# songhayeong/aes-fhe

Measured on AMD Instinct MI355X. Metric: AES-128 blocks/sec (homomorphic full round) at N=2^16, L=30; 1/2/4/8 MI355X, higher is better.
Workload: dtype u64

## Files before the change

### aes-fhe_amd/csrc/engine.hip

```cpp
#include <hip/hip_runtime.h>

#include <algorithm>
#include <atomic>
#include <cstdarg>
#include <cstdlib>
#include <cstdio>
#include <cstring>
#include <map>
#include <unordered_map>
#include <memory>
#include <mutex>
#include <string>
#include <vector>

#include "../../include/aesfhe.h"
#include "kernels_ops.h"
#include "ntt256f.h"
#include "ks_fused.h"
#include "bconv_mfma.h"
#include "bconv_cols.h"
#include "basis_tables.h"
#include "bsgs_plan.h"
#include "operands.h"
#include "arena.h"
// ... 824 lines not shown
extern "C" void aesfhe_key_free(aesfhe_key* k) {
    if (!k) return;
    aesfhe_engine* e = k->eng;
    e->pool.put(k->d, k->bytes);
    delete k;
    engine_unref(e);
}
extern "C" int aesfhe_key_info(const aesfhe_key* k, int32_t* kind, uint64_t* g) {
    *kind = k->kind;
    *g = k->galois;
    return 0;
}
extern "C" uint64_t aesfhe_galois_elt(int32_t logN, int64_t rot, int32_t conj) {
    u64 M = 2ULL << logN, n = 1ULL << (logN - 1);
    if (conj) return M - 1;
    int64_t r = rot % (int64_t)n;
    if (r < 0) r += (int64_t)n;
    u64 ex = (n - (u64)r) % n;
    return h_powmod(5, ex, M);
}

static aesfhe_key* key_new(aesfhe_engine* e, int kind, size_t words) {
    auto* k = new aesfhe_key;
    k->eng = e;
    e->refs++;
    k->kind = kind;
    k->galois = 0;
    k->keyseed = 0;
    k->bytes = words * 8;
    k->d = (u64*)pool_get(e, k->bytes);
    return k;
}

static void sample_small_ntt(aesfhe_engine* e, u64* dst, int nprimes, u64 key, int kind) {
    Span s = span_s(dst, 0, nprimes, std::min(nprimes, e->Lp1), 0, e->Lp1);
    s.pstride = (long)nprimes * e->N;
    hipLaunchKernelGGL(k_sample_small, dim3((e->N / 8 + 255) / 256), dim3(256), 0, e->stream, s, e->ck, key, kind, e->q, e->logN, e->Lp1, nprimes);
    ntt(e, s, s, nprimes, false);
}

extern "C" int aesfhe_key_secret(aesfhe_engine* e, uint64_t seed, aesfhe_key** out) {
    API_BEGIN
    aesfhe_key* k = key_new(e, 0, (size_t)e->np * e->N);
    k->keyseed = derive(e->seed, seed);
    sample_small_ntt(e, k->d, e->np, derive(k->keyseed, 1), 0);
    *out = k;
    API_END
}

extern "C" int aesfhe_key_public(aesfhe_engine* e, const aesfhe_key* sk, aesfhe_key** out) {
    API_BEGIN
    if (!sk || sk->kind != 0) throw_err(AESFHE_EARG, "public key needs a secret key");
    const int N = e->N, nq = e->Lp1;
    aesfhe_key* k = key_new(e, 1, (size_t)2 * nq * N);
    k->keyseed = sk->keyseed;
    u64* b = k->d;
    u64* a = k->d + (size_t)nq * N;
    Span sa = span_s(a, 0, nq, nq, 0, e->Lp1);
    hipLaunchKernelGGL(k_sample_uniform, dim3((N / 8 + 255) / 256, nq), dim3(256), 0, e->stream, sa, e->ck, derive(sk->keyseed, 2), e->q, e->logN, e->Lp1);
    Tmp et(e, (size_t)nq * N);
    sample_small_ntt(e, et.p, nq, derive(sk->keyseed, 3), 1);
    hipLaunchKernelGGL(k_key_combine, dim3(N / 256, nq), dim3(256), 0, e->stream, a, sk->d, et.p, (const u64*)nullptr, (const u64*)nullptr, 0, 0, b, e->q, e->qinv, e->logN);
    HIPC(hipGetLastError());
    *out = k;
    API_END
}

static aesfhe_key* make_ksk_t(aesfhe_engine* e, const u64* starget, u64 keyseed, const u64* sprime, int kind,
                              u64 g, u64 salt) {
    const int N = e->N, np = e->np;
    aesfhe_key* k = key_new(e, kind, (size_t)e->dnum * 2 * np * N);
    k->galois = g;
    k->keyseed = keyseed;
    k->ndig = e->dnum;
    u64 base = derive(derive(keyseed, 4 + (u64)kind), g);
    if (salt) base = derive(base, salt);
    Tmp et(e, (size_t)np * N);
    for (int d = 0; d < e->dnum; d++) {
        u64* kb = k->d + ((size_t)d * 2 + 0) * np * N;
        u64* ka = k->d + ((size_t)d * 2 + 1) * np * N;
        Span sa = span_s(ka, 0, np, e->Lp1, 0, e->Lp1);
        hipLaunchKernelGGL(k_sample_uniform, dim3((N / 8 + 255) / 256, np), dim3(256), 0, e->stream, sa, e->ck, derive(base, 2 * (u64)d), e->q, e->logN, e->Lp1);
        sample_small_ntt(e, et.p, np, derive(base, 2 * (u64)d + 1), 1);
        int lo = d * e->A, hi = std::min(lo + e->A, e->Lp1);
        hipLaunchKernelGGL(k_key_combine, dim3(N / 256, np), dim3(256), 0, e->stream, (const u64*)ka, starget, et.p, sprime, e->pmod, lo, hi, kb, e->q, e->qinv, e->logN);
    }
    HIPC(hipGetLastError());
    return k;
}
static aesfhe_key* make_ksk(aesfhe_engine* e, const aesfhe_key* sk, const u64* sprime, int kind, u64 g,
                            u64 salt = 0) {
    return make_ksk_t(e, sk->d, sk->keyseed, sprime, kind, g, salt);
}

extern "C" int aesfhe_key_relin(aesfhe_engine* e, const aesfhe_key* sk, aesfhe_key** out) {
    API_BEGIN
    if (!sk || sk->kind != 0) throw_err(AESFHE_EARG, "relinearization key needs a secret key");
    Tmp s2(e, (size_t)e->np * e->N);
    hipLaunchKernelGGL(k_square, dim3(e->N / 256, e->np), dim3(256), 0, e->stream, sk->d, s2.p, e->q, e->qinv, e->logN);
    *out = make_ksk(e, sk, s2.p, 2, 0);
    API_END
}

extern "C" int aesfhe_key_galois(aesfhe_engine* e, const aesfhe_key* sk, uint64_t g, aesfhe_key** out) {
    API_BEGIN
    if (!sk || sk->kind != 0) throw_err(AESFHE_EARG, "galois key needs a secret key");
    if (!(g & 1) || g >= 2ULL * e->N) throw_err(AESFHE_EARG, "bad galois element");
    Tmp sg(e, (size_t)e->np * e->N);
    Span src = span_s(sk->d, 0, e->np, e->Lp1, 0, e->Lp1), dst = span_s(sg.p, 0, e->np, e->Lp1, 0, e->Lp1);
    hipLaunchKernelGGL(k_galois, dim3(e->N / 256, e->np), dim3(256), 0, e->stream, src, dst, (u64)g, e->logN, e->Lp1);
    *out = make_ksk(e, sk, sg.p, 3, g);
    API_END
}

extern "C" int aesfhe_key_galois_hoisted(aesfhe_engine* e, const aesfhe_key* sk, uint64_t g, aesfhe_key** out) {
    API_BEGIN
    if (!sk || sk->kind != 0) throw_err(AESFHE_EARG, "galois key needs a secret key");
    if (!(g & 1) || g >= 2ULL * e->N) throw_err(AESFHE_EARG, "bad galois element");
    const u64 M = 2ULL * e->N;
    u64 ginv = 1;
// ... 75 lines not shown
    const size_t per = c->bytes / c->B;
    HIPC(hipMemcpyAsync(dst, (const char*)c->d + per * start, per * count, hipMemcpyDeviceToDevice, e->stream));
    HIPC(hipStreamSynchronize(e->stream));
    API_END
}
extern "C" int aesfhe_ct_import_device(aesfhe_engine* e, const void* src, int32_t B, int32_t np, int32_t level,
                                       aesfhe_ct** out) {
    API_BEGIN
    if (!src || B < 1 || np < 1 || np > 3 || level < 0 || level > e->L) throw_err(AESFHE_EARG, "bad shape");
    CtPtr c = ct_new(e, B, np, level);
    HIPC(hipMemcpyAsync(c->d, src, c->bytes, hipMemcpyDeviceToDevice, e->stream));
    HIPC(hipStreamSynchronize(e->stream));
    *out = c.release();
    API_END
}

static size_t key_words(const aesfhe_engine* e, int kind) {
    switch (kind) {
        case 0: return (size_t)e->np * e->N;
        case 1: return (size_t)2 * e->Lp1 * e->N;
        case 2: case 3: case 5: return (size_t)e->dnum * 2 * e->np * e->N;
        default: return 0;
    }
}
extern "C" int aesfhe_key_export(aesfhe_engine* e, const aesfhe_key* k, int32_t* kind, uint64_t* galois,
                                 uint64_t* keyseed, int64_t* words, uint64_t* out) {
    API_BEGIN
    if (!k) throw_err(AESFHE_EARG, "null key");
    *kind = k->kind;
    *galois = k->galois;
    *keyseed = k->keyseed;
    *words = (int64_t)(k->bytes / 8);
    if (out) {
        HIPC(hipMemcpyAsync(out, k->d, k->bytes, hipMemcpyDeviceToHost, e->stream));
        HIPC(hipStreamSynchronize(e->stream));
    }
    API_END
}
extern "C" int aesfhe_key_import(aesfhe_engine* e, int32_t kind, uint64_t galois, uint64_t keyseed,
                                 const uint64_t* in, int64_t words, aesfhe_key** out) {
    API_BEGIN
    size_t want = key_words(e, kind);
    if (!in || !want) throw_err(AESFHE_EARG, "unknown key kind %d", kind);
    int ndig = 0;
    if (kind == 2 || kind == 3 || kind == 5) {
        const size_t dw = (size_t)2 * e->np * e->N;
        if (words > 0 && (size_t)words % dw == 0 && (size_t)words / dw >= 1 && (size_t)words / dw <= (size_t)e->dnum)
            want = (size_t)words, ndig = (int)((size_t)words / dw);
    }
    if ((size_t)words != want) throw_err(AESFHE_EARG, "key of kind %d needs %zu words, got %lld", kind, want, (long long)words);
    aesfhe_key* k = key_new(e, kind, want);
    k->galois = galois;
    k->keyseed = keyseed;
    k->ndig = ndig;
    HIPC(hipMemcpyAsync(k->d, in, want * 8, hipMemcpyHostToDevice, e->stream));
    HIPC(hipStreamSynchronize(e->stream));
    *out = k;
    API_END
}
extern "C" int aesfhe_key_trim(aesfhe_engine* e, aesfhe_key* k, int32_t max_level) {
    API_BEGIN
    if (!k || k->ndig < 1) throw_err(AESFHE_EARG, "only switching keys (relinearization, galois, hoisted rotation) can be trimmed");
    if (max_level < 0 || max_level > e->L) throw_err(AESFHE_EARG, "bad level %d", max_level);
    const int nd = (max_level + 1 + e->A - 1) / e->A;
    if (nd < k->ndig) {
        const size_t bytes = (size_t)nd * 2 * e->np * e->N * 8;
        u64* d = (u64*)pool_get(e, bytes);
        HIPC(hipMemcpyAsync(d, k->d, bytes, hipMemcpyDeviceToDevice, e->stream));
        e->pool.put(k->d, k->bytes);
        k->d = d;
        k->bytes = bytes;
        k->ndig = nd;
    }
    API_END
}
static CtPtr ct_copy_new(aesfhe_engine* e, const aesfhe_ct* c) {
    CtPtr r = ct_new(e, c->B, c->np, c->level);
    HIPC(hipMemcpyAsync(r->d, c->d, c->bytes, hipMemcpyDeviceToDevice, e->stream));
    r->is_zero = c->is_zero;
    return r;
}
extern "C" int aesfhe_ct_copy(aesfhe_engine* e, const aesfhe_ct* c, aesfhe_ct** out) {
    API_BEGIN
    *out = ct_copy_new(e, c).release();
    API_END
}
extern "C" int aesfhe_ct_slice(aesfhe_engine* e, const aesfhe_ct* c, int32_t start, int32_t count, aesfhe_ct** out) {
    API_BEGIN
// ... 698 lines not shown
    a.scs = acs;
    a.dst = dst;
    a.dbs = 2 * kN;
    a.dcs = kN;
    a.nc = 2;
    a.ns = e->K + r;
    a.s_nq = r;
    a.s_q0 = lk + 1;
    a.s_p0 = e->Lp1;
    a.sinvf = ysrc ? nullptr : t.invf;
    a.einv = t.einv;
    a.nt = lk + 1;
    a.skip0 = lk + 1;
    a.skipn = 0;
    a.tl_l = lk;
    a.Lp1 = e->Lp1;
    a.tab = t.tab;
    a.corr = t.corr;
    a.pc = e->bc_pc;
    a.qall = e->q;
    a.qinvall = e->qinv;
    return a;
}

template <bool VC>
static void launch_bconv_cols_t(aesfhe_engine* e, const BconvArgs& a, int nz, int nslots) {
    const int nstep = (nslots + 3) / 4, ntile = (a.nt + 3) / 4;
    if (e->logN != 16 || nstep < 1 || nstep > 4 || ntile < 1 || (16 * nz) % 8)
        throw_err(AESFHE_EUNSUPPORTED, "fused base conversion of %d slots to %d targets", nslots, a.nt);
    if (!a.src || !a.dst || !a.tab || !a.corr || !a.pc || (VC && !a.einv))
        throw_err(AESFHE_EUNSUPPORTED, "fused base conversion with a missing table");
    const dim3 g((unsigned)(16 * nz * ntile));
    const Tabs T = e->tabs();
#define BCC(S) hipLaunchKernelGGL((k_bconv_cols<S, true, VC, 1>), g, dim3(256), 0, e->stream, a, T, ntile)
    switch (nstep) {
        case 1: BCC(1); break;
        case 2: BCC(2); break;
        case 3: BCC(3); break;
        default: BCC(4); break;
    }
#undef BCC
    HIPC(hipGetLastError());
}
static void launch_bconv_cols(aesfhe_engine* e, const BconvArgs& a, int nz) { launch_bconv_cols_t<false>(e, a, nz, a.ns); }

static std::vector<unsigned short> bsgs_block_order(int logN, const std::vector<u64>& gal) {
    std::vector<unsigned short> ord;
    if (!aesfhe::bsgs_block_order(logN, std::vector<uint64_t>(gal.begin(), gal.end()), ord))
        throw_err(AESFHE_EUNSUPPORTED, "bsgs block order is not a permutation");
    return ord;
}

static int ks_beta(const aesfhe_engine* e, int l) {
    const int beta = (l + 1 + e->A - 1) / e->A;
    if (beta > 12) throw_err(AESFHE_EUNSUPPORTED, "more than 12 key-switch digits");
    return beta;
}
static void check_key_digits(aesfhe_engine* e, const aesfhe_key* k, int l) {
    if (k && k->ndig > 0 && ks_beta(e, l) > k->ndig)
        throw_err(AESFHE_ELEVEL, "key trimmed to %d digits cannot switch at level %d (%d digits)", k->ndig, l, ks_beta(e, l));
}

static void ks_modup(aesfhe_engine* e, const u64* d, long dbs, int B, int l, u64* ext, bool cols_only = false,
                     const Opnd* pa = nullptr, const Opnd* pb = nullptr, const u64* fac = nullptr) {
    const int N = e->N, K = e->K, ne = l + 1 + K;
    const long lN = (long)(l + 1) * N, neN = (long)ne * N;
    const int beta = ks_beta(e, l);
// ... 1281 lines not shown
```

### aes-fhe_amd/csrc/ext/engine_ext.hip

```cpp
#include "../engine.hip"

#include "../../../include/aesfhe_ext.h"
#include "kernels_expand.h"
#include "kernels_lincomb_int.h"
#include "kernels_ptb.h"
#include "kernels_wire.h"

struct aesfhe_ptb {
    aesfhe_engine* eng;
    int B, level;
    u64* d;
    size_t bytes;
};

static const int kMaxGridZ = 65535;

extern "C" int aesfhe_ptb_create_device(aesfhe_engine* e, const int64_t* co, int32_t B, int32_t level, aesfhe_ptb** out) {
    API_BEGIN
    if (!e || !out) throw_err(AESFHE_EARG, "null argument");
    if (!co || ((uintptr_t)co & 15)) throw_err(AESFHE_EARG, "coefficient buffer must be a 16-byte aligned device pointer");
    if (level < 0 || level > e->L) throw_err(AESFHE_EARG, "bad plaintext level");
    if (B < 1 || B > kMaxGridZ) throw_err(AESFHE_EARG, "plaintext batch %d not in 1..%d", B, kMaxGridZ);
    const int N = e->N, nl = level + 1;
    struct PtbFree {
// ... 257 lines not shown
                           (const u64*)e->q, e->logN, (unsigned long long*)flag.p);
    }
    HIPC(hipGetLastError());
    u64 bad = 0;
    HIPC(hipMemcpyAsync(&bad, flag.p, 8, hipMemcpyDeviceToHost, e->stream));
    HIPC(hipStreamSynchronize(e->stream));
    if (bad) throw_err(AESFHE_EARG, "blob holds a residue that is not below its prime");
}

extern "C" int aesfhe_key_pack(aesfhe_engine* e, const aesfhe_key* k, const aesfhe_key* target, const uint8_t* seed, void* dst,
                               int64_t* bytes) {
    API_BEGIN
    if (!e || !k || !bytes) throw_err(AESFHE_EARG, "null argument");
    if (k->eng != e) throw_err(AESFHE_EARG, "key of another engine");
    if (target) {
        if (!seed) throw_err(AESFHE_EARG, "seeded packing needs 32 seed bytes");
        if (k->kind == 0) throw_err(AESFHE_EARG, "a secret key has no mask to seed");
        if (target->eng != e || target->kind != 0) throw_err(AESFHE_EARG, "seeded packing needs the secret key the rows are encrypted under");
    }
    const WireDims d = wire_dims(e);
    WireHeader h = wire_header_of(e, d);
    h.type = kWireKey, h.kind = k->kind, h.ndig = (uint32_t)k->ndig, h.galois = k->galois, h.keyseed = k->keyseed;
    h.npoly = k->kind == 0 ? 1 : 2;
    h.level = (k->kind == 1 ? e->Lp1 : e->np) - 1;
    WireShape s;
    if (!wire_pack_begin(e, d, h, s, seed, target != nullptr, dst, bytes)) return AESFHE_OK;
    if ((size_t)s.groups * s.polys * s.nl * e->N * 8 != k->bytes) throw_err(AESFHE_EARG, "key block of %zu bytes does not match its kind", k->bytes);
    u64 gal = 1;
    if (target && k->kind == 5) {
        const u64 M = 2ULL * e->N;
        for (u64 x = 1;; x = x * k->galois % M)
            if (x * k->galois % M == 1) { gal = x; break; }
    }
    wire_pack_run(e, h, s, k->d, target ? target->d : nullptr, gal, dst);
    API_END
}

extern "C" int aesfhe_ct_pack(aesfhe_engine* e, const aesfhe_ct* c, const aesfhe_key* sk, const uint8_t* seed, void* dst, int64_t* bytes) {
    API_BEGIN
    if (!e || !c || !bytes) throw_err(AESFHE_EARG, "null argument");
    if (c->eng != e) throw_err(AESFHE_EARG, "ciphertext of another engine");
    const bool seeded = sk != nullptr && !c->is_zero;
    if (sk) {
        if (!seed) throw_err(AESFHE_EARG, "seeded packing needs 32 seed bytes");
        if (sk->eng != e || sk->kind != 0) throw_err(AESFHE_EARG, "seeded packing needs the secret key");
        if (seeded && c->np != 2) throw_err(AESFHE_EDEGREE, "Input ciphertext should have 2 polynomials");
    }
    const WireDims d = wire_dims(e);
    WireHeader h = wire_header_of(e, d);
    h.type = kWireCt, h.batch = c->B, h.npoly = c->np, h.level = c->level, h.zero = c->is_zero ? 1 : 0;
    WireShape s;
    if (!wire_pack_begin(e, d, h, s, seed, seeded, dst, bytes)) return AESFHE_OK;
    wire_pack_run(e, h, s, c->d, seeded ? sk->d : nullptr, 1, dst);
    API_END
}

static void wire_unpack_begin(const aesfhe_engine* e, const void* src, int64_t bytes, uint32_t type, WireHeader& h, WireShape& s) {
    if (e->logN < kWireMinLogN) throw_err(AESFHE_EARG, "the wire format needs N >= 1024");
    const std::string err = wire_parse((const uint8_t*)src, bytes, wire_dims(e), h, s);
    if (!err.empty()) throw_err(AESFHE_EARG, "cannot unpack: %s", err.c_str());
    if (h.type != type) throw_err(AESFHE_EARG, "the blob holds a %s", h.type == kWireKey ? "key" : "ciphertext");
}

extern "C" int aesfhe_key_unpack(aesfhe_engine* e, const void* src, int64_t bytes, aesfhe_key** out) {
    API_BEGIN
    if (!e || !src || !out) throw_err(AESFHE_EARG, "null argument");
    WireHeader h;
    WireShape s;
    wire_unpack_begin(e, src, bytes, kWireKey, h, s);
    struct KeyFree {
        void operator()(aesfhe_key* k) const { aesfhe_key_free(k); }
    };
    std::unique_ptr<aesfhe_key, KeyFree> k(key_new(e, h.kind, (size_t)s.groups * s.polys * s.nl * e->N));
    k->galois = h.galois, k->keyseed = h.keyseed, k->ndig = (int)h.ndig;
    wire_unpack_run(e, h, s, src, k->d);
    *out = k.release();
    API_END
}

extern "C" int aesfhe_ct_unpack(aesfhe_engine* e, const void* src, int64_t bytes, aesfhe_ct** out) {
    API_BEGIN
    if (!e || !src || !out) throw_err(AESFHE_EARG, "null argument");
    WireHeader h;
    WireShape s;
    wire_unpack_begin(e, src, bytes, kWireCt, h, s);
    if (h.zero) {
        *out = ct_zero_new(e, h.batch, h.npoly, h.level).release();
        return AESFHE_OK;
    }
    CtPtr c = ct_new(e, h.batch, h.npoly, h.level);
    wire_unpack_run(e, h, s, src, c->d);
    *out = c.release();
    API_END
}
```

### aes-fhe_amd/csrc/kernels.h

```cpp
#pragma once
#include <hip/hip_runtime.h>

#include <cstdint>

#define AESFHE_HD __host__ __device__
#include "ckks_host.h"

namespace aesfhe {

constexpr int kMaxPrimes = 96;
constexpr double kBigPrime = 4398046511104.0;

__device__ __forceinline__ u64 add_m(u64 a, u64 b, u64 q) {
    u64 s = a + b;
    return s >= q ? s - q : s;
}
__device__ __forceinline__ u64 sub_m(u64 a, u64 b, u64 q) { return a >= b ? a - b : a + q - b; }

__device__ __forceinline__ u64 fix_m(u64 r, u64 q) {
    int64_t s = (int64_t)r;
    s = s < 0 ? s + (int64_t)q : s;
    s = s >= (int64_t)q ? s - (int64_t)q : s;
    return (u64)s;
}

__device__ __forceinline__ double u2d(u64 a) {
    return __longlong_as_double((long long)(a | 0x4330000000000000ULL)) - 4503599627370496.0;
}
__device__ __forceinline__ u64 rint_u(double x_times, double scale) {
    return (u64)__double_as_longlong(__builtin_fma(x_times, scale, 4503599627370496.0)) & 0xFFFFFFFFFFFFFULL;
}

__device__ __forceinline__ u64 mul_m(u64 a, u64 b, u64 q, double qinv) {
    const u64 qh = rint_u(u2d(a) * u2d(b), qinv);
    return fix_m(a * b - qh * q, q);
}
__device__ __forceinline__ u64 mul_w(u64 a, u64 w, double wq, u64 q) {
    const u64 qh = rint_u(u2d(a), wq);
    int64_t r = (int64_t)(a * w - qh * q);
    r += (r >> 63) & (int64_t)q;
    return (u64)r;
}

constexpr double kMagic52 = 6755399441055744.0;
__device__ __forceinline__ double fmul_rem(double a, double w, double wq, double q) {
    const double p = a * w;
    const double pl = __builtin_fma(a, w, -p);
    const double qh = __builtin_rint(a * wq);
    const double u = __builtin_fma(-qh, q, p);
    return u + pl;
}
__device__ __forceinline__ double fmul_rem_r(double a, double w, double wq, double q) {
    return fmul_rem(a, w, wq, q);
}
__device__ __forceinline__ double fmul_remq(double a, double w, double qi, double q) {
    const double p = a * w;
    const double pl = __builtin_fma(a, w, -p);
    const double qh = __builtin_rint(p * qi);
    const double u = __builtin_fma(-qh, q, p);
    return u + pl;
}
// ... 196 lines not shown
```

### aes-fhe_amd/csrc/kernels_ops.h

```cpp
#pragma once
#include "kernels.h"

namespace aesfhe {

__device__ __forceinline__ u64 red_m(u64 x, u64 q, double qinv) {
    u64 qh = (u64)((double)x * qinv);
    return fix_m(x - qh * q, q);
}

struct Opnd {
    const u64* ptr;
    long bs;
    long ps;
    int np;
    int bmask = -1;
};

__device__ const u64 kZeroWord = 0;
__device__ __forceinline__ u64 opnd_get(const Opnd& o, int b, int p, int l, int k, int logN) {
    const bool has = o.ptr && p < o.np;
    return *(has ? o.ptr + (long)(b & o.bmask) * o.bs + (long)p * o.ps + ((long)l << logN) + k : &kZeroWord);
}

struct Out {
// ... 261 lines not shown

__global__ void k_rescale_finish_g(const u64* __restrict__ c, long cps, const u64* __restrict__ t,
                                   u64* const* __restrict__ outs, long ops, int np, int Bg, int l,
                                   const u64* __restrict__ qs, const u64* __restrict__ inv,
                                   const double* __restrict__ invf, int logN) {
    const int k = blockIdx.x * blockDim.x + threadIdx.x;
    const int i = blockIdx.y, P = blockIdx.z;
    const int g = P / (Bg * np), rem = P - g * Bg * np;
    const u64 q = qs[i];
    u64 cv = c[(long)P * cps + ((long)i << logN) + k];
    u64 tv = t[(((long)P * l + i) << logN) + k];
    outs[g][(long)rem * ops + ((long)i << logN) + k] = mul_w(sub_m(cv, tv, q), inv[i], invf[i], q);
}

template <int BM>
__global__ void k_ks_inner_all(const u64* __restrict__ d, long dbs, const u64* __restrict__ ext,
                               long exs, long exj, const u64* __restrict__ key, long kdig,
                               long kcomp, u64* __restrict__ acc, long abs_, long acs, int B,
                               int beta, int K, int l, const u64* __restrict__ qall,
                               const double* __restrict__ qinvall, int Lp1, Opnd addend,
                               const double* __restrict__ pmodf, int logN, int accum) {
    const int k = blockIdx.x * blockDim.x + threadIdx.x;
    const int t = blockIdx.y;
    const int pid = t <= l ? t : Lp1 + (t - l - 1);
    const double q = (double)qall[pid];
    const double qi = qinvall[pid];
    const int own = t <= l ? t / K : -1;
    double kb[BM], ka[BM];
#pragma unroll
    for (int j = 0; j < BM; j++) {
        kb[j] = ka[j] = 0.0;
        if (j < beta) {
            const long ko = (long)j * kdig + ((long)pid << logN) + k;
            kb[j] = u2d(key[ko]);
            ka[j] = u2d(key[ko + kcomp]);
        }
    }
#pragma unroll 4
    for (int bb = 0; bb < B; bb++) {
        double s0 = 0.0, s1 = 0.0;
#pragma unroll
        for (int j = 0; j < BM; j++) {
            if (j < beta) {
                const double e = u2d((j == own) ? d[(long)bb * dbs + ((long)t << logN) + k]
                                                : ext[(long)j * exj + (long)bb * exs + ((long)t << logN) + k]);
                s0 += fmul_remq(e, kb[j], qi, q);
                s1 += fmul_remq(e, ka[j], qi, q);
                if ((j & 3) == 3) {
                    s0 = fred(s0, q, qi);
                    s1 = fred(s1, q, qi);
                }
            }
        }
        if (pmodf && t <= l) {
            const double f = pmodf[t], w = tw_w(f, q);
            s0 = fred(s0, q, qi) + fmul_rem(u2d(opnd_get(addend, bb, 0, t, k, logN)), w, f, q);
            s1 = fred(s1, q, qi) + fmul_rem(u2d(opnd_get(addend, bb, 1, t, k, logN)), w, f, q);
        }
        u64* a0 = acc + (long)bb * abs_ + ((long)t << logN) + k;
        if (accum) {
            s0 += u2d(a0[0]);
            s1 += u2d(a0[acs]);
        }
        a0[0] = fcanon(s0, q, qi);
        a0[acs] = fcanon(s1, q, qi);
    }
}

template <int BM, int KC>
__global__ void k_ks_inner_multi(const u64* __restrict__ d, long dbs, const u64* __restrict__ ext,
                                 long exs, long exj, const u64* const* __restrict__ keys, int nk, long kdig,
                                 long kcomp, u64* const* __restrict__ accs, long abs_, long acs, int B,
                                 int beta, int K, int l, const u64* __restrict__ qall,
                                 const double* __restrict__ qinvall, int Lp1, Opnd addend,
                                 const double* __restrict__ pmodf, int logN) {
    const int k = blockIdx.x * blockDim.x + threadIdx.x;
    const int t = blockIdx.y;
    const int pid = t <= l ? t : Lp1 + (t - l - 1);
    const double q = (double)qall[pid];
    const double qi = qinvall[pid];
    const int own = t <= l ? t / K : -1;
    const bool pm = pmodf && t <= l;
    const double f = pm ? pmodf[t] : 0.0, fw = pm ? tw_w(f, q) : 0.0;
    for (int i0 = 0; i0 < nk; i0 += KC) {
        double kb[KC][BM], ka[KC][BM];
#pragma unroll
        for (int ii = 0; ii < KC; ii++) {
#pragma unroll
            for (int j = 0; j < BM; j++) {
                const bool ok = i0 + ii < nk && j < beta;
                const u64* kp = keys[ok ? i0 + ii : 0] + (long)j * kdig + ((long)pid << logN) + k;
                kb[ii][j] = u2d(*(ok ? kp : &kZeroWord));
                ka[ii][j] = u2d(*(ok ? kp + kcomp : &kZeroWord));
            }
        }
#pragma unroll 1
        for (int bb = 0; bb < B; bb++) {
            double e[BM];
#pragma unroll
            for (int j = 0; j < BM; j++)
                e[j] = u2d(*(j >= beta ? &kZeroWord
                             : (j == own) ? d + (long)bb * dbs + ((long)t << logN) + k
                                          : ext + (long)j * exj + (long)bb * exs + ((long)t << logN) + k));
            double ad0 = 0.0, ad1 = 0.0;
            if (pm) {
                ad0 = fmul_rem(u2d(opnd_get(addend, bb, 0, t, k, logN)), fw, f, q);
                ad1 = fmul_rem(u2d(opnd_get(addend, bb, 1, t, k, logN)), fw, f, q);
            }
#pragma unroll
            for (int ii = 0; ii < KC; ii++) {
                if (i0 + ii >= nk) break;
                double s0 = 0.0, s1 = 0.0;
#pragma unroll
                for (int j = 0; j < BM; j++) {
                    if (j < beta) {
                        s0 += fmul_remq(e[j], kb[ii][j], qi, q);
                        s1 += fmul_remq(e[j], ka[ii][j], qi, q);
                        if ((j & 3) == 3) {
                            s0 = fred(s0, q, qi);
                            s1 = fred(s1, q, qi);
                        }
                    }
                }
                if (pm) {
                    s0 = fred(s0, q, qi) + ad0;
                    s1 = fred(s1, q, qi) + ad1;
// ... 142 lines not shown
            ulonglong2 w;
            w.x = v[e] >= 0 ? (u64)v[e] : q - (u64)(-v[e]);
            w.y = v[e + 1] >= 0 ? (u64)v[e + 1] : q - (u64)(-v[e + 1]);
            *(ulonglong2*)&out[k0 + e] = w;
        }
    }
}

__global__ void k_coeffs_res(const i64* __restrict__ co, u64* __restrict__ out, int nl,
                             const u64* __restrict__ qs, int logN) {
    const int k = blockIdx.x * blockDim.x + threadIdx.x;
    const int l = blockIdx.y, bb = blockIdx.z;
    const i64 v = co[((long)bb << logN) + k];
    const u64 q = qs[l];
    u64 r;
    if (v >= 0) r = (u64)v % q;
    else r = q - 1 - ((u64)(-(v + 1)) % q);
    out[(((long)bb * nl + l) << logN) + k] = r;
}

__global__ void k_key_combine(const u64* __restrict__ a, const u64* __restrict__ s,
                              const u64* __restrict__ e, const u64* __restrict__ sp,
                              const u64* __restrict__ pmod, int lo, int hi, u64* __restrict__ out,
                              const u64* __restrict__ qall, const double* __restrict__ qinvall,
                              int logN) {
    const int k = blockIdx.x * blockDim.x + threadIdx.x;
    const int pid = blockIdx.y;
    const long off = ((long)pid << logN) + k;
    const u64 q = qall[pid];
    const double qi = qinvall[pid];
    u64 v = add_m(sub_m(0, mul_m(a[off], s[off], q, qi), q), e[off], q);
    if (sp && pid >= lo && pid < hi) v = add_m(v, mul_m(pmod[pid], sp[off], q, qi), q);
    out[off] = v;
}

__global__ void k_enc_pk(const u64* __restrict__ vem, const u64* __restrict__ pk0,
                         const u64* __restrict__ pk1, u64* __restrict__ ct, int nl,
                         const u64* __restrict__ qs, const double* __restrict__ qinv, int logN) {
    const int k = blockIdx.x * blockDim.x + threadIdx.x;
    const int l = blockIdx.y, bb = blockIdx.z;
    const u64 q = qs[l];
    const double qi = qinv[l];
    const long lo = ((long)l << logN) + k;
    const long step = (long)nl << logN;
    const u64* base = vem + (long)bb * 4 * step + lo;
    u64 v = base[0], e0 = base[step], e1 = base[2 * step], m = base[3 * step];
    u64* c = ct + (long)bb * 2 * step + lo;
    c[0] = add_m(add_m(mul_m(v, pk0[lo], q, qi), e0, q), m, q);
    c[step] = add_m(mul_m(v, pk1[lo], q, qi), e1, q);
}

__global__ void k_enc_sk(const u64* __restrict__ vem, const u64* __restrict__ s,
                         u64* __restrict__ ct, int nl, const u64* __restrict__ qs,
                         const double* __restrict__ qinv, ChaKey K, const u64* __restrict__ keys, int logN) {
    const int k0 = (blockIdx.x * blockDim.x + threadIdx.x) * 8;
    if (k0 >= (1 << logN)) return;
    const int l = blockIdx.y, bb = blockIdx.z;
    const u64 q = qs[l];
    const double qi = qinv[l];
    const long step = (long)nl << logN;
    uint32_t o[16];
    chacha20_block(K, keys[bb], (((u64)l << logN) + k0) >> 3, o);
#pragma unroll
    for (int e = 0; e < 8; e++) {
        const long lo = ((long)l << logN) + k0 + e;
        const u64* base = vem + (long)bb * 4 * step + lo;
// ... 578 lines not shown
            for (int j = 0; j < GM; j++) {
                acc0[u][j] += fmul_remq(f0, wv[j], qi, q);
                acc1[u][j] += fmul_remq(f1, wv[j], qi, q);
            }
        }
    };
    int i = 0;
    if (!keys[0]) {
        double wv[GM], e0[BB], e1[BB];
#pragma unroll
        for (int j = 0; j < GM; j++) wv[j] = pt_word(j, 0);
#pragma unroll
        for (int u = 0; u < BB; u++) {
            e0[u] = isq ? fmul_rem(u2d(*(isq ? c0r[u] + k : &kZeroWord)), pw, pf, q) : 0.0;
            e1[u] = isq ? fmul_rem(u2d(*(isq ? c1r[u] + k : &kZeroWord)), pw, pf, q) : 0.0;
        }
        add_terms(e0, e1, wv);
        i = 1;
    }
    int nsum = 1;
#pragma unroll 1
    for (; i < nb; i += PB) {
        double kb[PB][BM], ka[PB][BM], x[PB][BB][BM], c0v[PB][BB], wv[PB][GM];
#pragma unroll
        for (int p = 0; p < PB; p++) {
            const int ii = min(i + p, nb - 1);
            const bool live = i + p < nb;
            const u64 g = gal[ii];
            const long src = __brev((unsigned)((((g * ek) & (M - 1)) - 1) >> 1)) >> (32 - logN);
            const u64* kp = keys[ii];
#pragma unroll
            for (int d = 0; d < BM; d++) {
                const u64* kk = kp + (long)min(d, beta - 1) * kdig + ((long)pid << logN) + src;
                kb[p][d] = u2d(kk[0]);
                ka[p][d] = u2d(kk[kcomp]);
            }
#pragma unroll
            for (int j = 0; j < GM; j++) wv[p][j] = live ? pt_word(j, ii) : 0.0;
#pragma unroll
            for (int u = 0; u < BB; u++) {
#pragma unroll
                for (int d = 0; d < BM; d++)
                    x[p][u][d] = u2d(*(d == own ? c1r[u] + src : er[u] + (long)min(d, beta - 1) * exj + src));
                c0v[p][u] = u2d(*(isq ? c0r[u] + src : &kZeroWord));
            }
        }
#pragma unroll
        for (int p = 0; p < PB; p++) {
            double e0[BB], e1[BB];
#pragma unroll
            for (int u = 0; u < BB; u++) {
                double a0 = isq ? fmul_rem(c0v[p][u], pw, pf, q) : 0.0, a1 = 0.0;
#pragma unroll
                for (int d = 0; d < BM; d++) {
                    if (d < beta) {
                        a0 += fmul_remq(x[p][u][d], kb[p][d], qi, q);
                        a1 += fmul_remq(x[p][u][d], ka[p][d], qi, q);
                        if ((d & 3) == 3) {
                            a0 = fred(a0, q, qi);
                            a1 = fred(a1, q, qi);
                        }
                    }
                }
                e0[u] = a0;
                e1[u] = a1;
            }
            add_terms(e0, e1, wv[p]);
        }
// ... 27 lines not shown
```

### aes-fhe_amd/csrc/ks_fused.h

```cpp
#pragma once
#include "kernels_ops.h"
#include "ntt256f.h"

#include <type_traits>

namespace aesfhe {

__device__ __forceinline__ int r8p(int e) { return e + (e >> 3); }

__device__ __forceinline__ void wave_lds_sync() {
    __builtin_amdgcn_fence(__ATOMIC_RELEASE, "wavefront");
    __builtin_amdgcn_wave_barrier();
    __builtin_amdgcn_fence(__ATOMIC_ACQUIRE, "wavefront");
}

template <bool BIG>
using KsBig = std::integral_constant<bool, BIG>;
template <class Big>
__device__ __forceinline__ void row_ntt8_stages(double (&x)[8], double* sr, int L, int rt, const double* W, double q,
                                                double qi, Big big);
__device__ __forceinline__ void row_ntt8_fwd(double (&x)[8], const u64* rp, double* sr, int L, int rt,
                                             const double* W, double q, double qi, bool big) {
#pragma unroll
    for (int r = 0; r < 8; r++) x[r] = ld_d(&rp[L + 32 * r]);
// ... 93 lines not shown
    const int eb = 32 * (L >> 2) + (L & 3);
#pragma unroll
    for (int r = 0; r < 8; r++) x[r] = sr[r8p(eb + 4 * r)];
#pragma unroll
    for (int st = 5; st >= 3; st--) {
        const int ml = 1 << st, h = 4 >> (st - 3), nj = ml >> 3;
        const int base = ml + (L >> 2) * nj;
#pragma unroll
        for (int j = 0; j < nj; j++) {
            const double w = W[base + j];
#pragma unroll
            for (int k = 0; k < h; k++) gs_f<BIG>(x[j * 2 * h + k], x[j * 2 * h + k + h], w, q, qi);
        }
    }
    wave_lds_sync();
#pragma unroll
    for (int r = 0; r < 8; r++) sr[r8p(eb + 4 * r)] = x[r];
    wave_lds_sync();
#pragma unroll
    for (int r = 0; r < 8; r++) x[r] = sr[r8p(L + 32 * r)];
#pragma unroll
    for (int st = 2; st >= 0; st--) {
        const int ml = 1 << st, h = 4 >> st;
#pragma unroll
        for (int j = 0; j < ml; j++) {
            const double w = W[ml + j];
#pragma unroll
            for (int k = 0; k < h; k++) gs_f<BIG>(x[j * 2 * h + k], x[j * 2 * h + k + h], w, q, qi);
        }
    }
    wave_lds_sync();
}

template <bool FMA, bool HAS_C, bool BIG>
__device__ __forceinline__ void ks_prod_prologue(double (&a0)[8], double (&a1)[8], const u64* kp, long kcomp,
                                                 const u64* xa, long aps, const u64* xb, long bps, const u64* xc,
                                                 long cps, double wv, double f, double fal, double fC, double fK,
                                                 double q, double qi) {
    static_assert(FMA || !HAS_C, "the addend ciphertext belongs to the multiply-add form");
    double x0[8], x1[8], y0[8], y1[8], kb[8], ka[8];
#pragma unroll
    for (int r = 0; r < 8; r++) {
        x0[r] = u2d(xa[32 * r]);
        x1[r] = u2d(xa[aps + 32 * r]);
        y0[r] = u2d(xb[32 * r]);
        y1[r] = u2d(xb[bps + 32 * r]);
        if constexpr (!FMA) {
            kb[r] = u2d(kp[32 * r]);
            ka[r] = u2d(kp[32 * r + kcomp]);
        }
    }
#pragma unroll
    for (int r = 0; r < 8; r++) {
        if constexpr (FMA) {
            kb[r] = u2d(kp[32 * r]);
            ka[r] = u2d(kp[32 * r + kcomp]);
        }
        double p0 = fmul_remq(x0[r], y0[r], qi, q);
        double p1 = fmul_remq(x0[r], y1[r], qi, q) + fmul_remq(x1[r], y0[r], qi, q);
        double p2 = fmul_remq(x1[r], y1[r], qi, q);
        if constexpr (FMA) {
            p0 = fmul_remq(p0, fal, qi, q) + fK;
            p1 = fmul_remq(p1, fal, qi, q);
            p2 = fmul_remq(p2, fal, qi, q);
            if constexpr (HAS_C) {
                p0 += fmul_remq(u2d(xc[32 * r]), fC, qi, q);
                p1 += fmul_remq(u2d(xc[cps + 32 * r]), fC, qi, q);
            }
        }
        a0[r] = fmul_rem(p0, wv, f, q) + fmul_remq(p2, kb[r], qi, q);
        a1[r] = fmul_rem(p1, wv, f, q) + fmul_remq(p2, ka[r], qi, q);
        if constexpr (BIG) {
            a0[r] = fred(a0[r], q, qi);
            a1[r] = fred(a1[r], q, qi);
        }
    }
}

struct KsFin {
    const u64* conv;
    long cbs, cps;
    u64* out;
    long obs, ops;
    const double* dinvf;
    Opnd2 add;
};
template <int G, int R = 256, bool PROD = false, int EPI = 0>
__global__ __launch_bounds__(256, 4) void k_nttf_rows_ks(const u64* __restrict__ d, long dbs,
                                                      const u64* __restrict__ ext, long exs, long exj,
                                                      const u64* __restrict__ key, long kdig, long kcomp,
                                                      u64* __restrict__ acc, long abs_, long acs, int B,
                                                      int beta, int K, int l, int ne, Tabs T, Opnd addend,
                                                      const double* __restrict__ pmodf, int accum, Opnd pb,
                                                      const u64* __restrict__ fac, Opnd pc, int t0, int nt,
                                                      KsFin fin) {
    static_assert(G == 1 && !PROD && EPI == 0, "the accumulating giants' kernel: the other forms are k_nttf_rows_ks_p's");
    __shared__ double s[8 * 288 + 8 * 256];
    const int nbg = (B + G - 1) / G;
    const int id = blockIdx.x, x8 = id & 7, rest = id >> 3;
    const int b0 = (rest % nbg) * G, pair = (rest / nbg) * 8 + x8;
    constexpr int RB = R / 8;
    constexpr int LOGN = R == 256 ? 16 : 17;
    const int tq = pair / RB, rb = pair - tq * RB;
    if (tq >= nt) return;
    const int t = t0 + tq;
    const int pid = t <= l ? t : T.Lp1 + (t - l - 1);
    const int own = t <= l ? t / K : -1;
    const int tid = threadIdx.x, L = tid & 31, rl = tid >> 5;
// ... 15 lines not shown
    const long roff = ((long)t << LOGN) + (long)row * 256 + L;
    double a0[G][8], a1[G][8];
#pragma unroll
    for (int g = 0; g < G; g++) {
        const int bb = b0 + g;
#pragma unroll
        for (int r = 0; r < 8; r++) a0[g][r] = a1[g][r] = 0.0;
        if (bb >= B) continue;
        if (pmodf && t <= l && addend.ptr) {
            const double f = pmodf[t], w = tw_w(f, q);
            const u64* xa = addend.ptr + (long)bb * addend.bs + roff;
            if (addend.np > 0) {
#pragma unroll
                for (int r = 0; r < 8; r++) a0[g][r] = fmul_rem(u2d(xa[32 * r]), w, f, q);
            }
            if (addend.np > 1) {
#pragma unroll
                for (int r = 0; r < 8; r++) a1[g][r] = fmul_rem(u2d(xa[addend.ps + 32 * r]), w, f, q);
            }
        }
        if (accum) {
            const u64* o0 = acc + (long)bb * abs_ + roff;
#pragma unroll
            for (int r = 0; r < 8; r++) {
                a0[g][r] = fred(a0[g][r] + u2d(o0[32 * r]), q, qi);
                a1[g][r] = fred(a1[g][r] + u2d(o0[acs + 32 * r]), q, qi);
            }
        }
    }
    int nsum = 0;
#pragma unroll 1
    for (int j = 0; j < beta; j++) {
        const u64* kp = key + (long)j * kdig + ((long)pid << LOGN) + (long)row * 256 + L;
        u64 kbw[8], kaw[8];
#pragma unroll
        for (int r = 0; r < 8; r++) {
            kbw[r] = kp[32 * r];
            kaw[r] = kp[32 * r + kcomp];
        }
#pragma unroll
        for (int g = 0; g < G; g++) {
            const int bb = b0 + g;
            if (bb >= B) break;
            double v[8];
            if (j == own) {
                const u64* dp = d + (long)bb * dbs + roff;
#pragma unroll
                for (int r = 0; r < 8; r++) v[r] = u2d(dp[32 * r]);
            } else {
                row_ntt8_fwd(v, ext + (long)j * exj + (long)bb * exs + ((long)t << LOGN) + (long)row * 256, sr, L, 1,
                             tw, q, qi, big);
            }
#pragma unroll
            for (int r = 0; r < 8; r++) {
                const double kb = u2d(kbw[r]), ka = u2d(kaw[r]);
                a0[g][r] += fmul_remq(v[r], kb, qi, q);
                a1[g][r] += fmul_remq(v[r], ka, qi, q);
            }
        }
        if (big && (++nsum & 3) == 0) {
#pragma unroll
            for (int g = 0; g < G; g++)
#pragma unroll
                for (int r = 0; r < 8; r++) {
                    a0[g][r] = fred(a0[g][r], q, qi);
                    a1[g][r] = fred(a1[g][r], q, qi);
                }
        }
    }
#pragma unroll
    for (int g = 0; g < G; g++) {
        const int bb = b0 + g;
        if (bb >= B) break;
        u64* o0 = acc + (long)bb * abs_ + roff;
#pragma unroll
        for (int r = 0; r < 8; r++) {
            __builtin_nontemporal_store(fcanon(a0[g][r], q, qi), &o0[32 * r]);
            __builtin_nontemporal_store(fcanon(a1[g][r], q, qi), &o0[acs + 32 * r]);
        }
    }
}

typedef __attribute__((address_space(3))) void ks_lds_void;
__device__ __forceinline__ void ks_dma_rows(const u64* g, double* lds_wave, int lane) {
#pragma unroll
    for (int k = 0; k < 4; k++)
        __builtin_amdgcn_global_load_lds((const void*)(g + 128 * k + 2 * lane), (ks_lds_void*)(lds_wave + 128 * k), 16, 0, 0);
}
__device__ __forceinline__ void ks_dma_wait() {
    asm volatile("s_waitcnt vmcnt(0)" ::: "memory");
// ... 30 lines not shown
    const double q = (double)T.q[pid], qi = T.qinv[pid];
    const double* W = T.psid + ((long)pid << LOGN);
    double* sr = s + rl * 288;
    double* tw = s + 8 * 288 + rl * 256;
    double* ebw = s + 8 * 288 + 8 * 256 + w * 512;
    const double* er = ebw + (rl & 1) * 256;
    const long woff = ((long)t << LOGN) + (long)(rb * 8 + 2 * w) * 256;
    auto next_digit = [&](int j) { return j + 1 == own ? j + 2 : j + 1; };
    int jn = next_digit(-1);
    if (jn < beta) ks_dma_rows(ext + (long)jn * exj + (long)bb * exs + woff, ebw, lane);
#pragma unroll
    for (int m = 0; m < 8; m++) {
        const int e = L + 32 * m;
        if (e > 0) {
            const int ml = 1 << (31 - __clz(e));
            tw[e] = W[(long)ml * (R + row) + (e - ml)];
        }
    }
    const long roff = ((long)t << LOGN) + (long)row * 256 + L;
    auto body = [&](auto big) {
        constexpr bool BIG = decltype(big)::value;
        double a0[8], a1[8];
#pragma unroll
        for (int r = 0; r < 8; r++) a0[r] = a1[r] = 0.0;
        if (PROD && t <= l) {
            const double f = pmodf[t], wv = tw_w(f, q);
            const u64* kp = key + (long)own * kdig + ((long)pid << LOGN) + (long)row * 256 + L;
            const u64* xa = addend.ptr + (long)(bb & addend.bmask) * addend.bs + roff;
            const u64* xb = pb.ptr + (long)(bb & pb.bmask) * pb.bs + roff;
            const u64* xc = pc.ptr ? pc.ptr + (long)(bb & pc.bmask) * pc.bs + roff : xb;
            if (fac) {
                const double fal = (double)fac[3 * t], fC = (double)fac[3 * t + 1], fK = (double)fac[3 * t + 2];
                if (pc.ptr)
                    ks_prod_prologue<true, true, BIG>(a0, a1, kp, kcomp, xa, addend.ps, xb, pb.ps, xc, pc.ps, wv, f, fal, fC,
                                                      fK, q, qi);
                else
                    ks_prod_prologue<true, false, BIG>(a0, a1, kp, kcomp, xa, addend.ps, xb, pb.ps, xc, pc.ps, wv, f, fal,
                                                       fC, fK, q, qi);
            } else {
                ks_prod_prologue<false, false, BIG>(a0, a1, kp, kcomp, xa, addend.ps, xb, pb.ps, xc, pc.ps, wv, f, 0.0, 0.0,
                                                    0.0, q, qi);
            }
        } else if (!PROD) {
            if (pmodf && t <= l && addend.ptr) {
                const double f = pmodf[t], wv = tw_w(f, q);
                const u64* xa = addend.ptr + (long)bb * addend.bs + roff;
                if (addend.np > 0) {
#pragma unroll
                    for (int r = 0; r < 8; r++) a0[r] = fmul_rem(u2d(xa[32 * r]), wv, f, q);
                }
                if (addend.np > 1) {
#pragma unroll
                    for (int r = 0; r < 8; r++) a1[r] = fmul_rem(u2d(xa[addend.ps + 32 * r]), wv, f, q);
                }
            }
            if (own >= 0 && own < beta) {
                const u64* kp = key + (long)own * kdig + ((long)pid << LOGN) + (long)row * 256 + L;
                const u64* dp = d + (long)bb * dbs + roff;
#pragma unroll
                for (int r = 0; r < 8; r++) {
                    const double v = u2d(dp[32 * r]), kb = u2d(kp[32 * r]), ka = u2d(kp[32 * r + kcomp]);
                    a0[r] += fmul_remq(v, kb, qi, q);
                    a1[r] += fmul_remq(v, ka, qi, q);
                }
            }
        }
        if (accum) {
            const u64* o0 = acc + (long)bb * abs_ + roff;
#pragma unroll
            for (int r = 0; r < 8; r++) {
                a0[r] = fred(a0[r] + u2d(o0[32 * r]), q, qi);
                a1[r] = fred(a1[r] + u2d(o0[acs + 32 * r]), q, qi);
            }
        } else if (BIG) {
#pragma unroll
            for (int r = 0; r < 8; r++) {
                a0[r] = fred(a0[r], q, qi);
                a1[r] = fred(a1[r], q, qi);
            }
        }
        wave_lds_sync();
        int nsum = 0;
        const long coff = ((long)t << LOGN) + (long)(rb * 8 + 2 * w) * 256;
#pragma unroll 1
        while (jn < beta) {
            const int j = jn;
            ks_dma_wait();
            double v[8];
#pragma unroll
            for (int r = 0; r < 8; r++) v[r] = er[L + 32 * r];
            ks_lds_reads_done();
            jn = next_digit(j);
            if constexpr (FIN)
                ks_dma_rows(jn < beta ? ext + (long)jn * exj + (long)bb * exs + woff : fin.conv + (long)bb * fin.cbs + coff,
                            ebw, lane);
            else if (jn < beta) ks_dma_rows(ext + (long)jn * exj + (long)bb * exs + woff, ebw, lane);
            const u64* kp = key + (long)j * kdig + ((long)pid << LOGN) + (long)row * 256 + L;
            u64 kbw[8], kaw[8];
#pragma unroll
            for (int r = 0; r < 8; r++) {
                kbw[r] = kp[32 * r];
                kaw[r] = kp[32 * r + kcomp];
            }
            row_ntt8_stages(v, sr, L, 1, tw, q, qi, big);
#pragma unroll
            for (int r = 0; r < 8; r++) {
                const double kb = u2d(kbw[r]), ka = u2d(kaw[r]);
                a0[r] += fmul_remq(v[r], kb, qi, q);
                a1[r] += fmul_remq(v[r], ka, qi, q);
            }
            if (BIG && (++nsum & 3) == 0) {
#pragma unroll
                for (int r = 0; r < 8; r++) {
                    a0[r] = fred(a0[r], q, qi);
                    a1[r] = fred(a1[r], q, qi);
                }
            }
        }
        if constexpr (FIN) {
            const double f = fin.dinvf[t], wv = tw_w(f, q);
            if (beta == 0 || next_digit(-1) >= beta)
                ks_dma_rows(fin.conv + (long)bb * fin.cbs + coff, ebw, lane);
#pragma unroll 1
            for (int c = 0; c < 2; c++) {
                ks_dma_wait();
                double cv[8];
#pragma unroll
                for (int r = 0; r < 8; r++) cv[r] = er[L + 32 * r];
                ks_lds_reads_done();
                if (c == 0) ks_dma_rows(fin.conv + (long)bb * fin.cbs + fin.cps + coff, ebw, lane);
                row_ntt8_stages(cv, sr, L, 1, tw, q, qi, big);
                const u64* ap = fin.add.ptr && c < fin.add.np ? fin.add.ptr + (long)bb * fin.add.bs + (long)c * fin.add.ps + roff
                                                              : nullptr;
                u64* op = fin.out + (long)bb * fin.obs + (long)c * fin.ops + roff;
                double v[8];
#pragma unroll
                for (int r = 0; r < 8; r++) {
                    double a = c ? a1[r] : a0[r];
                    if constexpr (BIG) a = fred(a, q, qi);
                    v[r] = fmul_rem(a - cv[r], wv, f, q);
                }
                if (ap) {
// ... 36 lines not shown
```

Baseline: 286,900.

## Store switching keys at rest as f64 bit patterns to skip per-use conversion

Switching keys (relin, galois, hoisted rotation) are converted once after creation or import into f64 bit patterns. Key-switch kernels can then reinterpret the loaded words directly instead of doing u2d (an OR plus a subtract) on every load. Export and wire-pack convert the keys back to u64 words in a temporary buffer. The change also drops the extra BIG-mode reductions in the prologue, and the non-VC bconv_cols launch now uses template variant 2. Together these touch key storage format, the kernels and the serialization paths, so any path that reads key->d as raw u64 without going through the new conversion would be wrong.

```diff
diff --git a/aes-fhe_amd/csrc/engine.hip b/aes-fhe_amd/csrc/engine.hip
--- a/aes-fhe_amd/csrc/engine.hip
+++ b/aes-fhe_amd/csrc/engine.hip
@@ -880,6 +880,22 @@
     return k;
 }
 
+static bool key_rests_f64(const aesfhe_key* k) { return k->kind == 2 || k->kind == 3 || k->kind == 5; }
+static void key_to_rest(aesfhe_engine* e, aesfhe_key* k) {
+    if (!key_rests_f64(k)) return;
+    const long n = (long)(k->bytes / 8);
+    hipLaunchKernelGGL(k_key_rest, dim3((unsigned)((n + 255) / 256)), dim3(256), 0, e->stream, k->d, n);
+    HIPC(hipGetLastError());
+}
+static const u64* key_u64_words(aesfhe_engine* e, const aesfhe_key* k, Tmp& tmp) {
+    if (!key_rests_f64(k)) return k->d;
+    const long n = (long)(k->bytes / 8);
+    tmp = Tmp(e, (size_t)n);
+    hipLaunchKernelGGL(k_key_words, dim3((unsigned)((n + 255) / 256)), dim3(256), 0, e->stream, (const u64*)k->d, tmp.p, n);
+    HIPC(hipGetLastError());
+    return tmp.p;
+}
+
 static void sample_small_ntt(aesfhe_engine* e, u64* dst, int nprimes, u64 key, int kind) {
     Span s = span_s(dst, 0, nprimes, std::min(nprimes, e->Lp1), 0, e->Lp1);
     s.pstride = (long)nprimes * e->N;
@@ -934,6 +950,7 @@
         hipLaunchKernelGGL(k_key_combine, dim3(N / 256, np), dim3(256), 0, e->stream, (const u64*)ka, starget, et.p, sprime, e->pmod, lo, hi, kb, e->q, e->qinv, e->logN);
     }
     HIPC(hipGetLastError());
+    key_to_rest(e, k);
     return k;
 }
 static aesfhe_key* make_ksk(aesfhe_engine* e, const aesfhe_key* sk, const u64* sprime, int kind, u64 g,
@@ -1075,7 +1092,8 @@
     *keyseed = k->keyseed;
     *words = (int64_t)(k->bytes / 8);
     if (out) {
-        HIPC(hipMemcpyAsync(out, k->d, k->bytes, hipMemcpyDeviceToHost, e->stream));
+        Tmp words;
+        HIPC(hipMemcpyAsync(out, key_u64_words(e, k, words), k->bytes, hipMemcpyDeviceToHost, e->stream));
         HIPC(hipStreamSynchronize(e->stream));
     }
     API_END
@@ -1097,6 +1115,7 @@
     k->keyseed = keyseed;
     k->ndig = ndig;
     HIPC(hipMemcpyAsync(k->d, in, want * 8, hipMemcpyHostToDevice, e->stream));
+    key_to_rest(e, k);
     HIPC(hipStreamSynchronize(e->stream));
     *out = k;
     API_END
@@ -1861,7 +1880,7 @@
         throw_err(AESFHE_EUNSUPPORTED, "fused base conversion with a missing table");
     const dim3 g((unsigned)(16 * nz * ntile));
     const Tabs T = e->tabs();
-#define BCC(S) hipLaunchKernelGGL((k_bconv_cols<S, true, VC, 1>), g, dim3(256), 0, e->stream, a, T, ntile)
+#define BCC(S) hipLaunchKernelGGL((k_bconv_cols<S, true, VC, VC ? 1 : 2>), g, dim3(256), 0, e->stream, a, T, ntile)
     switch (nstep) {
         case 1: BCC(1); break;
         case 2: BCC(2); break;
diff --git a/aes-fhe_amd/csrc/ext/engine_ext.hip b/aes-fhe_amd/csrc/ext/engine_ext.hip
--- a/aes-fhe_amd/csrc/ext/engine_ext.hip
+++ b/aes-fhe_amd/csrc/ext/engine_ext.hip
@@ -313,7 +313,8 @@
         for (u64 x = 1;; x = x * k->galois % M)
             if (x * k->galois % M == 1) { gal = x; break; }
     }
-    wire_pack_run(e, h, s, k->d, target ? target->d : nullptr, gal, dst);
+    Tmp words;
+    wire_pack_run(e, h, s, key_u64_words(e, k, words), target ? target->d : nullptr, gal, dst);
     API_END
 }
 
@@ -355,6 +356,7 @@
     std::unique_ptr<aesfhe_key, KeyFree> k(key_new(e, h.kind, (size_t)s.groups * s.polys * s.nl * e->N));
     k->galois = h.galois, k->keyseed = h.keyseed, k->ndig = (int)h.ndig;
     wire_unpack_run(e, h, s, src, k->d);
+    key_to_rest(e, k.get());
     *out = k.release();
     API_END
 }
diff --git a/aes-fhe_amd/csrc/kernels.h b/aes-fhe_amd/csrc/kernels.h
--- a/aes-fhe_amd/csrc/kernels.h
+++ b/aes-fhe_amd/csrc/kernels.h
@@ -27,6 +27,7 @@
 __device__ __forceinline__ double u2d(u64 a) {
     return __longlong_as_double((long long)(a | 0x4330000000000000ULL)) - 4503599627370496.0;
 }
+__device__ __forceinline__ double key_d(const u64* p) { return __longlong_as_double((long long)*p); }
 __device__ __forceinline__ u64 rint_u(double x_times, double scale) {
     return (u64)__double_as_longlong(__builtin_fma(x_times, scale, 4503599627370496.0)) & 0xFFFFFFFFFFFFFULL;
 }
diff --git a/aes-fhe_amd/csrc/kernels_ops.h b/aes-fhe_amd/csrc/kernels_ops.h
--- a/aes-fhe_amd/csrc/kernels_ops.h
+++ b/aes-fhe_amd/csrc/kernels_ops.h
@@ -317,8 +317,8 @@
         kb[j] = ka[j] = 0.0;
         if (j < beta) {
             const long ko = (long)j * kdig + ((long)pid << logN) + k;
-            kb[j] = u2d(key[ko]);
-            ka[j] = u2d(key[ko + kcomp]);
+            kb[j] = key_d(&key[ko]);
+            ka[j] = key_d(&key[ko + kcomp]);
         }
     }
 #pragma unroll 4
@@ -375,8 +375,8 @@
             for (int j = 0; j < BM; j++) {
                 const bool ok = i0 + ii < nk && j < beta;
                 const u64* kp = keys[ok ? i0 + ii : 0] + (long)j * kdig + ((long)pid << logN) + k;
-                kb[ii][j] = u2d(*(ok ? kp : &kZeroWord));
-                ka[ii][j] = u2d(*(ok ? kp + kcomp : &kZeroWord));
+                kb[ii][j] = key_d(ok ? kp : &kZeroWord);
+                ka[ii][j] = key_d(ok ? kp + kcomp : &kZeroWord);
             }
         }
 #pragma unroll 1
@@ -585,6 +585,15 @@
     u64 v = add_m(sub_m(0, mul_m(a[off], s[off], q, qi), q), e[off], q);
     if (sp && pid >= lo && pid < hi) v = add_m(v, mul_m(pmod[pid], sp[off], q, qi), q);
     out[off] = v;
+}
+
+__global__ void k_key_rest(u64* __restrict__ d, long n) {
+    const long i = (long)blockIdx.x * blockDim.x + threadIdx.x;
+    if (i < n) d[i] = (u64)__double_as_longlong(u2d(d[i]));
+}
+__global__ void k_key_words(const u64* __restrict__ d, u64* __restrict__ out, long n) {
+    const long i = (long)blockIdx.x * blockDim.x + threadIdx.x;
+    if (i < n) out[i] = (u64)__double_as_longlong(key_d(&d[i]) + 4503599627370496.0) & 0xFFFFFFFFFFFFFULL;
 }
 
 __global__ void k_enc_pk(const u64* __restrict__ vem, const u64* __restrict__ pk0,
@@ -1229,8 +1238,8 @@
 #pragma unroll
             for (int d = 0; d < BM; d++) {
                 const u64* kk = kp + (long)min(d, beta - 1) * kdig + ((long)pid << logN) + src;
-                kb[p][d] = u2d(kk[0]);
-                ka[p][d] = u2d(kk[kcomp]);
+                kb[p][d] = key_d(&kk[0]);
+                ka[p][d] = key_d(&kk[kcomp]);
             }
 #pragma unroll
             for (int j = 0; j < GM; j++) wv[p][j] = live ? pt_word(j, ii) : 0.0;
diff --git a/aes-fhe_amd/csrc/ks_fused.h b/aes-fhe_amd/csrc/ks_fused.h
--- a/aes-fhe_amd/csrc/ks_fused.h
+++ b/aes-fhe_amd/csrc/ks_fused.h
@@ -149,7 +149,7 @@
     wave_lds_sync();
 }
 
-template <bool FMA, bool HAS_C, bool BIG>
+template <bool FMA, bool HAS_C>
 __device__ __forceinline__ void ks_prod_prologue(double (&a0)[8], double (&a1)[8], const u64* kp, long kcomp,
                                                  const u64* xa, long aps, const u64* xb, long bps, const u64* xc,
                                                  long cps, double wv, double f, double fal, double fC, double fK,
@@ -163,15 +163,15 @@
         y0[r] = u2d(xb[32 * r]);
         y1[r] = u2d(xb[bps + 32 * r]);
         if constexpr (!FMA) {
-            kb[r] = u2d(kp[32 * r]);
-            ka[r] = u2d(kp[32 * r + kcomp]);
+            kb[r] = key_d(&kp[32 * r]);
+            ka[r] = key_d(&kp[32 * r + kcomp]);
         }
     }
 #pragma unroll
     for (int r = 0; r < 8; r++) {
         if constexpr (FMA) {
-            kb[r] = u2d(kp[32 * r]);
-            ka[r] = u2d(kp[32 * r + kcomp]);
+            kb[r] = key_d(&kp[32 * r]);
+            ka[r] = key_d(&kp[32 * r + kcomp]);
         }
         double p0 = fmul_remq(x0[r], y0[r], qi, q);
         double p1 = fmul_remq(x0[r], y1[r], qi, q) + fmul_remq(x1[r], y0[r], qi, q);
@@ -187,10 +187,6 @@
         }
         a0[r] = fmul_rem(p0, wv, f, q) + fmul_remq(p2, kb[r], qi, q);
         a1[r] = fmul_rem(p1, wv, f, q) + fmul_remq(p2, ka[r], qi, q);
-        if constexpr (BIG) {
-            a0[r] = fred(a0[r], q, qi);
-            a1[r] = fred(a1[r], q, qi);
-        }
     }
 }
 
@@ -272,11 +268,11 @@
 #pragma unroll 1
     for (int j = 0; j < beta; j++) {
         const u64* kp = key + (long)j * kdig + ((long)pid << LOGN) + (long)row * 256 + L;
-        u64 kbw[8], kaw[8];
+        double kbw[8], kaw[8];
 #pragma unroll
         for (int r = 0; r < 8; r++) {
-            kbw[r] = kp[32 * r];
-            kaw[r] = kp[32 * r + kcomp];
+            kbw[r] = key_d(&kp[32 * r]);
+            kaw[r] = key_d(&kp[32 * r + kcomp]);
         }
 #pragma unroll
         for (int g = 0; g < G; g++) {
@@ -293,9 +289,8 @@
             }
 #pragma unroll
             for (int r = 0; r < 8; r++) {
-                const double kb = u2d(kbw[r]), ka = u2d(kaw[r]);
-                a0[g][r] += fmul_remq(v[r], kb, qi, q);
-                a1[g][r] += fmul_remq(v[r], ka, qi, q);
+                a0[g][r] += fmul_remq(v[r], kbw[r], qi, q);
+                a1[g][r] += fmul_remq(v[r], kaw[r], qi, q);
             }
         }
         if (big && (++nsum & 3) == 0) {
@@ -392,13 +387,13 @@
             if (fac) {
                 const double fal = (double)fac[3 * t], fC = (double)fac[3 * t + 1], fK = (double)fac[3 * t + 2];
                 if (pc.ptr)
-                    ks_prod_prologue<true, true, BIG>(a0, a1, kp, kcomp, xa, addend.ps, xb, pb.ps, xc, pc.ps, wv, f, fal, fC,
+                    ks_prod_prologue<true, true>(a0, a1, kp, kcomp, xa, addend.ps, xb, pb.ps, xc, pc.ps, wv, f, fal, fC,
                                                       fK, q, qi);
                 else
-                    ks_prod_prologue<true, false, BIG>(a0, a1, kp, kcomp, xa, addend.ps, xb, pb.ps, xc, pc.ps, wv, f, fal,
+                    ks_prod_prologue<true, false>(a0, a1, kp, kcomp, xa, addend.ps, xb, pb.ps, xc, pc.ps, wv, f, fal,
                                                        fC, fK, q, qi);
             } else {
-                ks_prod_prologue<false, false, BIG>(a0, a1, kp, kcomp, xa, addend.ps, xb, pb.ps, xc, pc.ps, wv, f, 0.0, 0.0,
+                ks_prod_prologue<false, false>(a0, a1, kp, kcomp, xa, addend.ps, xb, pb.ps, xc, pc.ps, wv, f, 0.0, 0.0,
                                                     0.0, q, qi);
             }
         } else if (!PROD) {
@@ -419,7 +414,7 @@
                 const u64* dp = d + (long)bb * dbs + roff;
 #pragma unroll
                 for (int r = 0; r < 8; r++) {
-                    const double v = u2d(dp[32 * r]), kb = u2d(kp[32 * r]), ka = u2d(kp[32 * r + kcomp]);
+                    const double v = u2d(dp[32 * r]), kb = key_d(&kp[32 * r]), ka = key_d(&kp[32 * r + kcomp]);
                     a0[r] += fmul_remq(v, kb, qi, q);
                     a1[r] += fmul_remq(v, ka, qi, q);
                 }
@@ -431,12 +426,6 @@
             for (int r = 0; r < 8; r++) {
                 a0[r] = fred(a0[r] + u2d(o0[32 * r]), q, qi);
                 a1[r] = fred(a1[r] + u2d(o0[acs + 32 * r]), q, qi);
-            }
-        } else if (BIG) {
-#pragma unroll
-            for (int r = 0; r < 8; r++) {
-                a0[r] = fred(a0[r], q, qi);
-                a1[r] = fred(a1[r], q, qi);
             }
         }
         wave_lds_sync();
@@ -456,18 +445,17 @@
                             ebw, lane);
             else if (jn < beta) ks_dma_rows(ext + (long)jn * exj + (long)bb * exs + woff, ebw, lane);
             const u64* kp = key + (long)j * kdig + ((long)pid << LOGN) + (long)row * 256 + L;
-            u64 kbw[8], kaw[8];
+            double kbw[8], kaw[8];
 #pragma unroll
             for (int r = 0; r < 8; r++) {
-                kbw[r] = kp[32 * r];
-                kaw[r] = kp[32 * r + kcomp];
+                kbw[r] = key_d(&kp[32 * r]);
+                kaw[r] = key_d(&kp[32 * r + kcomp]);
             }
             row_ntt8_stages(v, sr, L, 1, tw, q, qi, big);
 #pragma unroll
             for (int r = 0; r < 8; r++) {
-                const double kb = u2d(kbw[r]), ka = u2d(kaw[r]);
-                a0[r] += fmul_remq(v[r], kb, qi, q);
-                a1[r] += fmul_remq(v[r], ka, qi, q);
+                a0[r] += fmul_remq(v[r], kbw[r], qi, q);
+                a1[r] += fmul_remq(v[r], kaw[r], qi, q);
             }
             if (BIG && (++nsum & 3) == 0) {
 #pragma unroll
```

Measured after the change: 288,800, median of 6. Within noise of the previous version (+0.7%).
